# Research-Implementation/AudioVidSum-A-Multi-Modal-Approach-to-Video-Summarization

Measured on AMD Instinct MI355X. Metric: frames/sec end-to-end (extract+fuse+score), 224x224 + 16kHz, higher is better.
Workload: dtype f16x2; 1 GPU; configs[1]: SumMe-shape batch, 25 videos x ~1800 frames (45143 frames/GPU), visual-only resnet50 extractor (batch-stat BN, the reference's 4-frame BatchNorm micro-batches inside each video) + AVBiLSTM attention scorer + mean-threshold selection; frames_per_gpu=45143, videos_per_gpu=25, extractor=resnet50, frames_per_group=4, chunk_frames=16384, parallelism=videos sharded x1, no data-path collective, selected_frames_rank0=22823

## Files before the change

### audiovidsum-a-multi-modal-approach-to-video-summarization_amd/_abi.py

```python
import ctypes
import os
from ctypes import POINTER, c_char_p, c_double, c_float, c_int, c_int64, c_size_t, c_uint, c_void_p

import torch

_PKG_DIR = os.path.dirname(os.path.abspath(__file__))
STUDY = os.environ.get("AVS_STUDY_LIB") == "1"
_FLAVOUR = os.environ.get("AVS_STUDY_LIB")
LIB_PATH = os.path.join(_PKG_DIR, "lib", "libavsum_hip_study.so" if STUDY else
                        "libavsum_hip_fp16emu.so" if _FLAVOUR == "fp16emu" else "libavsum_hip.so")
HEADER_PATH = os.path.join(os.path.dirname(_PKG_DIR), "include", "avsum_hip.h")

AVS_F32, AVS_BF16, AVS_F32_ACC64, AVS_F32_SPLIT, AVS_F16X2 = 0, 1, 2, 3, 4
AVS_W_ROWS, AVS_W_KSTEP32 = 0, 1
TILE_AUTO, TILE_128, TILE_256, TILE_224, STAGING_GENERIC = 0, 1, 2, 3, 4
X_F16P8, Y_F16P8, RES_F16P8 = 1, 2, 4
LSTM_AUTO, LSTM_STREAM, LSTM_RESIDENT_20_8, LSTM_RESIDENT_16_8 = 0, 1, 2, 3
LSTM_SPLIT4 = 4
ACT_NONE, ACT_RELU = 0, 1
BIAS_NONE, BIAS_COL, BIAS_ROW = 0, 1, 2
E_UNSUPPORTED = -6


class AvsError(RuntimeError):
    pass


class ConvDesc(ctypes.Structure):
    _fields_ = [
        ("dtype", c_int),
        ("n", c_int), ("h", c_int), ("w", c_int),
        ("cin", c_int), ("kh", c_int), ("kw", c_int),
        ("sh", c_int), ("sw", c_int), ("ph", c_int), ("pw", c_int),
        ("ho", c_int), ("wo", c_int), ("cout", c_int),
        ("x_img_stride", c_int64), ("x_row_stride", c_int64), ("x_px_stride", c_int64),
        ("w_row_stride", c_int64), ("y_px_stride", c_int64),
        ("act", c_int), ("alpha", c_float), ("w_layout", c_int), ("variant", c_int), ("formats", c_int),
    ]


P = c_void_p
_SIGNATURES = {
    "avs_abi_version": (c_int, []),
    "avs_last_error": (c_char_p, []),
    "avs_device_info": (c_int, [c_int, POINTER(c_int), POINTER(c_int), POINTER(c_int64), c_char_p, c_int]),
    "avs_f16x2_pack_f32": (c_int, [P, P, c_int64, P]),
    "avs_f16x2_unpack_f32": (c_int, [P, P, c_int64, P]),
    "avs_f16p8_pack_f32": (c_int, [P, P, c_int64, P]),
# ... 77 lines not shown
    "avs_lstm_split_f32": (c_int, [P, P, c_int, c_int, c_uint, P, c_int, P, c_int64, c_int, P, P, P, c_size_t, c_uint, P]),
    "avs_lstm_bwd_split_f32": (c_int, [P, c_int64, c_int, P, P, P, c_int, c_int, c_uint, P, c_int, P, P, c_size_t, c_uint, P]),
    "avs_cdist_f64": (c_int, [P, c_int, P, c_int, c_int, P, P]),
    "avs_dtw_workspace_bytes": (c_int64, [c_int, c_int]),
    "avs_dtw_path_f64": (c_int, [P, c_int, c_int, P, c_int64, P, P, P, P]),
    "avs_gather_scale_f32": (c_int, [P, c_int64, c_int, P, P, c_int, P, P]),
}

_lib = None


def declared_symbols():
    import re
    text = open(HEADER_PATH).read()
    text = re.sub(r"/\*.*?\*/", "", text, flags=re.S)
    return sorted(set(re.findall(r"\b(avs_[a-z0-9_]+)\s*\(", text)))


def lib():
    global _lib
    if _lib is not None:
        return _lib
    if not os.path.exists(LIB_PATH):
        raise AvsError(
            f"{LIB_PATH} is missing: the HIP extension has not been built "
            "(run __graft_entry__.build() or `make -C <package>/csrc`). There is no CPU fallback."
        )
    handle = ctypes.CDLL(LIB_PATH)
    if STUDY:
        handle.avs_debug_flags.restype = None
        handle.avs_debug_flags.argtypes = [c_int]
        for name, args in (("avs_tune_short_reduction_bytes", [c_int]), ("avs_tune_tall_rule", [c_int, c_int]),
                           ("avs_tune_pipeline", [c_int]), ("avs_tune_bnlocal", [c_int]),
                           ("avs_tune_convbn_narrow", [c_int])):
            getattr(handle, name).restype = None
            getattr(handle, name).argtypes = args
    for name, (res, args) in _SIGNATURES.items():
        fn = getattr(handle, name)
        fn.restype = res
        fn.argtypes = args
    if handle.avs_abi_version() != 5:
        raise AvsError(f"ABI version mismatch: library reports {handle.avs_abi_version()}, binding expects 5")
    if STUDY and os.environ.get("AVS_TUNE_CONVBN_NARROW") is not None:
        handle.avs_tune_convbn_narrow(int(os.environ["AVS_TUNE_CONVBN_NARROW"]))
    if STUDY and os.environ.get("AVS_TUNE_PIPELINE") is not None:
        handle.avs_tune_pipeline(int(os.environ["AVS_TUNE_PIPELINE"]))
    _lib = handle
    return _lib


def check(status, what):
    if status != 0:
        msg = lib().avs_last_error()
        raise AvsError(f"{what} failed with status {status}: {msg.decode() if msg else ''}")


def device_info(dev=0):
    cu, clk, mem = c_int(), c_int(), c_int64()
    arch = ctypes.create_string_buffer(64)
    check(lib().avs_device_info(dev, ctypes.byref(cu), ctypes.byref(clk), ctypes.byref(mem), arch, 64),
          "avs_device_info")
    return {"cu_count": cu.value, "clock_khz": clk.value, "hbm_bytes": mem.value, "arch": arch.value.decode()}
```

### audiovidsum-a-multi-modal-approach-to-video-summarization_amd/csrc/igemm.hip

```cpp
#include "avs_internal.h"
#include "igemm_params.h"
#include <type_traits>

__device__ __attribute__((aligned(16))) unsigned int avs_zero16[4];

#ifdef AVS_STUDY
#define AVS_DEBUG_BIT(p, bit) ((p).debug & (bit))
#else
#define AVS_DEBUG_BIT(p, bit) 0
#endif

#define AVS_GLDS16(src, dst)                                                                        \
  __builtin_amdgcn_global_load_lds((const __attribute__((address_space(1))) void*)(src),            \
                                   (__attribute__((address_space(3))) void*)(dst), 16, 0, 0)

__device__ __forceinline__ void avs_split_bf16(const float4& p0, const float4& p1, bf16x8& hi, bf16x8& lo) {
  const float v[8] = {p0.x, p0.y, p0.z, p0.w, p1.x, p1.y, p1.z, p1.w};
  unsigned h[4], l[4];
#pragma unroll
  for (int j = 0; j < 4; ++j) {
    const unsigned short h0 = avs_f32_to_bf16(v[2 * j]), h1 = avs_f32_to_bf16(v[2 * j + 1]);
    const unsigned short l0 = avs_f32_to_bf16(v[2 * j] - avs_bf16_to_f32(h0));
    const unsigned short l1 = avs_f32_to_bf16(v[2 * j + 1] - avs_bf16_to_f32(h1));
    h[j] = (unsigned)h0 | ((unsigned)h1 << 16);
// ... 1414 lines not shown
            v = (float)(acc64[mt][nt][e] * (double)p.alpha) + bcol;
          else if constexpr (EPI == EPI_ANY)
            v = fmaf(acc[mt][nt][e], p.alpha, bcol);
          else if constexpr (EPI == EPI_BRELU)
            v = fmaxf(acc[mt][nt][e] + bcol, 0.f);
          else
            v = acc[mt][nt][e];
          if constexpr (EPI == EPI_ANY) {
            if (p.bias_mode == AVS_BIAS_ROW) v += bias[row];
            if (p.act == AVS_ACT_RELU) v = fmaxf(v, 0.f);
          }
          *reinterpret_cast<float*>(y + ((long long)row * p.ldc + col) * 4) = v;
        }
      }
    stats_fold();
  }
  }
}

#ifdef AVS_STUDY
static int g_debug_flags = 0;
extern "C" void avs_debug_flags(int flags) { g_debug_flags = flags; }
#endif
#ifdef AVS_STUDY
#define AVS_RULE static int
#else
#define AVS_RULE static constexpr int
#endif
AVS_RULE g_rowb_threshold_bytes = 2048;
AVS_RULE g_tall_min_tiles = 2048;
AVS_RULE g_tall_min_k_bytes = 1024;
AVS_RULE g_pipe3 = 1;
AVS_RULE g_bnlocal = 1;
static constexpr int AVS_RULE_AFFINE_128_MAX_K = 128;
#ifdef AVS_STUDY
extern "C" void avs_tune_short_reduction_bytes(int bytes) { g_rowb_threshold_bytes = bytes; }
extern "C" void avs_tune_tall_rule(int min_tiles, int min_k_bytes) {
  if (min_tiles > 0) g_tall_min_tiles = min_tiles;
  if (min_k_bytes >= 0) g_tall_min_k_bytes = min_k_bytes;
}
extern "C" void avs_tune_pipeline(int enabled) { g_pipe3 = enabled; }
extern "C" void avs_tune_bnlocal(int enabled) { g_bnlocal = enabled; }
#endif

static bool igemm_tap9_ok(const IgemmParams& p, int es) {
  return (p.variant & 3) != AVS_TILE_256 && p.KW == 3 && p.K == 9 * p.cin && p.sh == 1 && p.sw == 1 && p.ph == 1 && p.pw == 1 &&
         p.W <= 63 && p.HoWo == p.H * p.W && p.Wo == p.W && p.x_px_stride == p.cin &&
         p.x_row_stride == (long long)p.W * p.cin && p.x_img_stride == (long long)p.HoWo * p.cin && p.cin % (64 / es) == 0 &&
         (long long)(384 + 64) * p.cin * es < (1ll << 31);
}

static bool igemm_taps_ok(const IgemmParams& p) {
  if ((p.variant & 3) == AVS_TILE_256 || p.cin <= 0 || p.KW <= 0 || p.K % (p.cin * p.KW) != 0) return false;
  const int kh = p.K / (p.cin * p.KW);
  return kh * p.KW > 1 && kh * p.KW <= 32 && p.sh == 1 && p.sw == 1 && 2 * p.ph + 1 == kh && 2 * p.pw + 1 == p.KW &&
         p.HoWo == p.H * p.W && p.Wo == p.W && p.ph * p.W + p.pw <= 64 && p.x_px_stride >= p.cin &&
         p.x_row_stride == (long long)p.W * p.x_px_stride && p.x_img_stride == (long long)p.HoWo * p.x_px_stride &&
         p.cin % 16 == 0 && (long long)(384 + 64) * p.x_px_stride * 4 + (long long)p.cin * 4 < (1ll << 31);
}

#define AVS_LAUNCH_RET(K)                                     \
  do {                                                        \
    hipLaunchKernelGGL(K, grid, dim3(256), 0, stream, p);     \
    return true;                                              \
  } while (0)
template <int ES, int BN, bool ACC64, bool SP, int ROWB, bool PIPE, int WR, bool FK>
static bool igemm_dispatch_epi4(int epi, dim3 grid, hipStream_t stream, const IgemmParams& p) {
  if (p.in_scale) {
    if constexpr (ES == 4 && !ACC64 && SP && ROWB == 64 && PIPE && WR == 4 && FK) {
      if (p.split == 2 && epi == EPI_STATS && igemm_tap9_ok(p, ES))
        AVS_LAUNCH_RET((igemm_kernel<ES, BN, ACC64, SP, ROWB, EPI_STATS, PIPE, WR, FK, 2, true, false, true>));
    }
    return false;
  }
  if constexpr (ES == 2 && WR == 4) {
// ... 249 lines not shown
                    p.x_img_stride == (long long)p.HoWo * p.x_px_stride && p.x_px_stride % 16 == 0 &&
                    256 * p.x_px_stride * 3 + (long long)p.K * 3 < (1ll << 31),
                AVS_E_UNSUPPORTED,
                "%s: an AVS_F16P8 input is taken by avs_conv2d_nhwc_bnstats for 1x1 / stride-1 convolutions on dense rows, "
                "cin a multiple of 32 (>= 64), the input row stride a multiple of 16", who);
  }
  if (p.affine) {
    const int tile_mode = p.variant & 3;
    p.tall = (!narrow && (tile_mode == AVS_TILE_128 || (tile_mode == AVS_TILE_AUTO && p.K <= AVS_RULE_AFFINE_128_MAX_K))) ? 0 : 1;
    if (!p.tall && (long long)p.K * 4 > g_rowb_threshold_bytes) p.tall = 1;
  }
  const int tile_rows = p.tile_rows ? p.tile_rows : (p.tall ? 256 : 128);
  const long long tiles_m = ((long long)p.M + tile_rows - 1) / tile_rows;
  const long long total = tiles_m * p.tiles_n;
  AVS_REQUIRE(total < (1ll << 31), AVS_E_SHAPE, "%s: too many tiles", who);
  if (tiles_m_out) *tiles_m_out = tiles_m;
  if (plan_only) return AVS_OK;
  const bool spatial = !(p.ph == 0 && p.pw == 0 && (p.HoWo / p.Wo - 1) * p.sh + (p.K / (p.cin * p.KW)) - 1 < p.H &&
                         (p.Wo - 1) * p.sw + p.KW - 1 < p.W);
  p.lin_stride = -1;
  if (!spatial && p.KW == 1 && p.K == p.cin && p.sh == 1 && p.sw == 1) {
    if (p.HoWo == 1)
      p.lin_stride = p.x_img_stride;
    else if (p.x_row_stride == (long long)p.Wo * p.x_px_stride && p.x_img_stride == (long long)p.HoWo * p.x_px_stride)
      p.lin_stride = p.x_px_stride;
  }
  dim3 grid((unsigned)total, 1, (unsigned)batch);
  if (p.tile_rows && dtype == AVS_F16X2) {
    const bool fits = igemm_h2_local224_ok(p, dtype);
    AVS_REQUIRE(fits || p.cluster <= 1, AVS_E_UNSUPPORTED, "%s: the clustered form runs on the 224-row tile only", who);
    AVS_REQUIRE(fits || (p.variant & 3) != AVS_TILE_224, AVS_E_UNSUPPORTED,
                "%s: AVS_TILE_224 takes AVS_F16X2, groups of 193..224 rows, cout in multiples of 128, cin in multiples of 16", who);
    if (fits) {
      igemm_h2_local224_launch(p, spatial, grid, stream);
      AVS_CHECK_LAUNCH(who);
      return AVS_OK;
    }
  }
  bool launched;
  if (wide96) {
    launched = igemm_dispatch_brelu96(spatial, grid, stream, p);
  } else if (dtype == AVS_BF16) {
    launched = narrow ? igemm_dispatch<2, 64, false>(spatial, grid, stream, p) : igemm_dispatch<2, 128, false>(spatial, grid, stream, p);
  } else if (dtype == AVS_F32_ACC64) {
    launched = igemm_dispatch<4, 64, true>(spatial, grid, stream, p);
  } else {
    launched = narrow ? igemm_dispatch<4, 64, false>(spatial, grid, stream, p) : igemm_dispatch<4, 128, false>(spatial, grid, stream, p);
  }
  AVS_REQUIRE(launched, AVS_E_UNSUPPORTED,
              "%s: no kernel for this combination (dtype %d, %s tile, K = %d, N = %d, variant %d, %s%s%s): nothing was launched", who,
              dtype, p.tall ? "256-row" : "128-row", p.K, p.N, p.variant, p.affine ? "given-affine " : "", p.tile_rows ? "tile-local " : "",
              p.stat_part ? "statistics" : "");
  AVS_CHECK_LAUNCH(who);
  return AVS_OK;
}

static int conv_fill_params(const avs_conv_desc* d, const void* d_x, const void* d_w, const float* d_bias, void* d_y,
                            IgemmParams& p, const char* who) {
  AVS_REQUIRE(d != nullptr, AVS_E_ARG, "%s: null descriptor", who);
  AVS_REQUIRE(d->n >= 0 && d->h > 0 && d->w > 0 && d->cin > 0 && d->kh > 0 && d->kw > 0 && d->sh > 0 && d->sw > 0 &&
                  d->ph >= 0 && d->pw >= 0 && d->ho > 0 && d->wo > 0 && d->cout > 0,
              AVS_E_SHAPE, "%s: non-positive extent", who);
  AVS_REQUIRE((d->ho - 1) * d->sh - d->ph + d->kh - 1 < d->h + d->ph &&
                  (d->wo - 1) * d->sw - d->pw + d->kw - 1 < d->w + d->pw,
              AVS_E_SHAPE, "%s: output extent %dx%d exceeds what input %dx%d allows", who, d->ho, d->wo, d->h, d->w);
  const long long rows = (long long)d->n * d->ho * d->wo;
  AVS_REQUIRE(rows < (1ll << 31), AVS_E_SHAPE, "%s: %lld output pixels exceed int32", who, rows);
  p.x = (const char*)d_x;
  p.w = (const char*)d_w;
  p.y = (char*)d_y;
  p.bias = d_bias;
  p.M = (int)rows;
  p.N = d->cout;
  p.K = d->kh * d->kw * d->cin;
  p.HoWo = d->ho * d->wo;
  p.Wo = d->wo;
  p.H = d->h;
  p.W = d->w;
  p.cin = d->cin;
  p.KW = d->kw;
  p.sh = d->sh;
  p.sw = d->sw;
  p.ph = d->ph;
  p.pw = d->pw;
  p.x_img_stride = d->x_img_stride;
  p.x_row_stride = d->x_row_stride;
  p.x_px_stride = d->x_px_stride;
  p.ldb = d->w_row_stride;
  AVS_REQUIRE(d->w_layout == AVS_W_ROWS || d->w_layout == AVS_W_KSTEP32, AVS_E_ARG, "%s: bad w_layout %d", who,
              d->w_layout);
  p.w_kstep = d->w_layout == AVS_W_KSTEP32 ? 1 : 0;
  AVS_REQUIRE((d->variant & ~7) == 0, AVS_E_ARG, "%s: bad variant %d", who, d->variant);
  p.variant = d->variant;
  AVS_REQUIRE((d->formats & ~(AVS_X_F16P8 | AVS_Y_F16P8 | AVS_RES_F16P8)) == 0, AVS_E_ARG, "%s: bad formats %d", who, d->formats);
  AVS_REQUIRE(d->formats == 0 || d->dtype == AVS_F16X2, AVS_E_UNSUPPORTED, "%s: AVS_F16P8 operands belong to the AVS_F16X2 forms", who);
  p.x_p8 = (d->formats & AVS_X_F16P8) ? 1 : 0;
  p.y_p8 = (d->formats & AVS_Y_F16P8) ? 1 : 0;
  p.res_p8 = (d->formats & AVS_RES_F16P8) ? 1 : 0;
  AVS_REQUIRE(!p.w_kstep || (d->dtype != AVS_F32_ACC64 && p.K % (d->dtype == AVS_BF16 ? 32 : 16) == 0), AVS_E_UNSUPPORTED,
              "%s: the reduction-step-major weight layout needs a reduction that is a multiple of a 64-byte step (K = %d)",
              who, p.K);
  p.ldc = d->y_px_stride;
  p.alpha = d->alpha;
  p.act = d->act;
  p.bias_mode = d_bias ? AVS_BIAS_COL : AVS_BIAS_NONE;
  AVS_REQUIRE(p.ldb >= p.K, AVS_E_SHAPE, "%s: w_row_stride %lld < kh*kw*cin=%d", who, p.ldb, p.K);
  return AVS_OK;
}

extern "C" int avs_conv2d_nhwc(const avs_conv_desc* d, const void* d_x, const void* d_w, const float* d_bias,
                               void* d_y, avs_stream_t stream) {
  IgemmParams p{};
  int st = conv_fill_params(d, d_x, d_w, d_bias, d_y, p, "avs_conv2d_nhwc");
  if (st != AVS_OK) return st;
  return igemm_launch(d->dtype, p, 1, (hipStream_t)stream, "avs_conv2d_nhwc");
}

extern "C" int avs_conv2d_nhwc_split(const avs_conv_desc* d, const void* d_x, const void* d_w, const float* d_bias,
                                     void* d_y, int n_split, void* d_y2, int64_t y2_px_stride, int relu_cols,
                                     avs_stream_t stream) {
  const char* who = "avs_conv2d_nhwc_split";
  IgemmParams p{};
  int st = conv_fill_params(d, d_x, d_w, d_bias, d_y, p, who);
  if (st != AVS_OK) return st;
  AVS_REQUIRE(d->dtype == AVS_F16X2, AVS_E_UNSUPPORTED, "%s: built for AVS_F16X2", who);
// ... 342 lines not shown
```

### audiovidsum-a-multi-modal-approach-to-video-summarization_amd/csrc/igemm_params.h

```cpp
#pragma once
#include "avs_internal.h"

typedef __bf16 bf16x8 __attribute__((ext_vector_type(8)));
typedef float f32x16 __attribute__((ext_vector_type(16)));

struct IgemmParams {
  const char* x;
  const char* w;
  char* y;
  const float* bias;
  int M, N, K;
  int HoWo, Wo, H, W, cin, KW;
  int sh, sw, ph, pw;
  long long x_img_stride, x_row_stride, x_px_stride;
  long long ldb, ldc;
  long long sA, sB, sC, sBias;
  float alpha;
  int act, bias_mode;
  int tiles_n;
  float* stat_part;
  int stat_slots;
  int rows_per_group;
  long long lin_stride;
  const float* gamma;
  const float* beta;
  float eps;
  const char* residual;
  long long ldr;
  int split;
  int tall;
  int w_kstep;
  int tile_rows;
  int affine;
  const float* res_scale;
  const float* res_shift;
  int variant;
  int x_p8, y_p8, res_p8;
  char* y2;
  long long ldc2;
  int nsplit;
  int relu_cols;
  int cluster;
  unsigned epoch;
  unsigned long long* xchg;
  unsigned* xerr;
  const float* in_scale;
  const float* in_shift;
  int in_relu;
#ifdef AVS_STUDY
  int debug;
#endif
};

enum { EPI_PLAIN = 0, EPI_STATS = 1, EPI_ANY = 2, EPI_BRELU = 3, EPI_BNLOCAL = 5, EPI_AFFINE = 6 };
constexpr int BNLOCAL_MAX_GROUPS = 6;
constexpr int STATS_MIN_GROUP_ROWS = 64;

typedef unsigned u32x4 __attribute__((ext_vector_type(4)));
typedef unsigned u32x2 __attribute__((ext_vector_type(2)));
__device__ __forceinline__ void avs_pin(uint4& v) {
  u32x4 r = __builtin_bit_cast(u32x4, v);
  asm volatile("" : "+v"(r));
  v = __builtin_bit_cast(uint4, r);
}

__device__ __forceinline__ void avs_pin2(uint2& v) {
  u32x2 r = __builtin_bit_cast(u32x2, v);
  asm volatile("" : "+v"(r));
  v = __builtin_bit_cast(uint2, r);
}
__device__ __forceinline__ uint2 avs_lds_read_b64(unsigned byte_addr) {
  uint2 v;
  asm volatile("ds_read_b64 %0, %1" : "=v"(v) : "v"(byte_addr));
  return v;
}
__device__ __forceinline__ uint4 avs_lds_read_b128(unsigned byte_addr) {
  uint4 v;
  asm volatile("ds_read_b128 %0, %1" : "=v"(v) : "v"(byte_addr));
// ... 7 lines not shown
```

### audiovidsum-a-multi-modal-approach-to-video-summarization_amd/csrc/local224.hip

```cpp
#include "avs_internal.h"
#include "igemm_params.h"
#include <type_traits>
#include <utility>

namespace {
constexpr int L_ROWS = 224;
constexpr int L_MT = L_ROWS / 32;
constexpr int L_BN = 128;
constexpr int L_CPRR = 4;
constexpr int L_STEP = 16;
constexpr int L_BUF = (L_ROWS + L_BN) * L_CPRR;
constexpr int L_P = 32 + 8;
constexpr unsigned L_OOB = 0x80000000u;

template <int OFF>
__device__ __forceinline__ uint4 lds_read_b128_at(unsigned byte_addr) {
  uint4 v;
  asm volatile("ds_read_b128 %0, %1 offset:%2" : "=v"(v) : "v"(byte_addr), "n"(OFF));
  return v;
}
template <int... I>
__device__ __forceinline__ void read_blocks(uint4 (&f)[L_MT], unsigned addr, std::integer_sequence<int, I...>) {
  ((f[I] = lds_read_b128_at<I * 32 * 64>(addr)), ...);
}
}

template <bool SPATIAL>
__global__ __launch_bounds__(256, 2) void igemm_h2_local224_kernel(IgemmParams p) {
  __shared__ uint4 lds[3 * L_BUF];

  const unsigned nwg = gridDim.x, orig = blockIdx.x;
  const unsigned q = nwg >> 3, rr = nwg & 7, xcd = orig & 7;
  const unsigned wg = (xcd < rr ? xcd * (q + 1) : rr * (q + 1) + (xcd - rr) * q) + (orig >> 3);
  int tn = wg % p.tiles_n;
  int tm = wg / p.tiles_n;
  if (p.cluster > 1) {
    const unsigned c = (unsigned)p.cluster, tnn = (unsigned)p.tiles_n;
    const unsigned tiles_m = nwg / tnn;
    const unsigned full = (8u % c == 0u) ? (tiles_m / 8u) * 8u : 0u;
    if (orig < full * tnn) {
      const unsigned su = orig / (8u * tnn), l = orig - su * (8u * tnn);
      tn = (int)(l >> 3);
      tm = (int)(su * 8u + (l & 7u));
    } else {
      const unsigned o2 = orig - full * tnn, unit = c * tnn;
      const unsigned u = o2 / unit, l = o2 - u * unit;
      tn = (int)(l / c);
      tm = (int)(full + u * c + l % c);
    }
  }
  const int m0 = tm * p.tile_rows;
  const int n0 = tn * L_BN;
  const int used = m0 + p.tile_rows <= p.M ? p.tile_rows : p.M - m0;

  const char* __restrict__ x = p.x;
  const char* __restrict__ w = p.w;
  char* __restrict__ y = p.y;

  const int t = threadIdx.x;
  const int wave = __builtin_amdgcn_readfirstlane(t >> 6), lane = t & 63;
  const bool extra = wave < 2;
  const int c = t & (L_CPRR - 1);
  const int rb = t >> 2;
  const int cq = c ^ ((rb >> 2) & (L_CPRR - 1));

  unsigned amask[4], aoff[4], boff[2];
  int f_tap = 0, f_ci0 = 0, f_kw = 0;
  int f_koff = 0;
  int f_kb = 0;
  __amdgpu_buffer_rsrc_t a_rsrc, b_rsrc;
  {
    const int taps = p.K / p.cin;
    long long a_origin;
    int n_first = 0;
    if (p.lin_stride >= 0) {
      a_origin = (long long)m0 * p.lin_stride;
    } else {
      n_first = m0 / p.HoWo;
      a_origin = (long long)n_first * p.x_img_stride - (long long)p.ph * p.x_row_stride - (long long)p.pw * p.x_px_stride;
    }
    a_rsrc = __builtin_amdgcn_make_buffer_rsrc(const_cast<char*>(x) + a_origin * 4, 0, (int)L_OOB, 0x00020000);
    b_rsrc = __builtin_amdgcn_make_buffer_rsrc(
        const_cast<char*>(w) + (p.w_kstep ? (long long)n0 * 64 : (long long)n0 * p.ldb * 4), 0, (int)L_OOB, 0x00020000);
#pragma unroll
    for (int i = 0; i < 4; ++i) {
      unsigned mk = 0, off = L_OOB;
      const int r = rb + 64 * i;
      if (r < used) {
        const int m = m0 + r;
        if (p.lin_stride >= 0) {
          mk = ~0u;
          off = (unsigned)((long long)r * p.lin_stride * 4) + cq * 16;
        } else {
          const int n = m / p.HoWo;
          const int rem = m - n * p.HoWo;
          const int ho = rem / p.Wo;
          const int wo = rem - ho * p.Wo;
          const int hi0 = ho * p.sh - p.ph, wi0 = wo * p.sw - p.pw;
          if constexpr (SPATIAL) {
            for (int tp = 0; tp < taps; ++tp) {
              const int th = tp / p.KW, tw = tp - th * p.KW;
              if ((unsigned)(hi0 + th) < (unsigned)p.H && (unsigned)(wi0 + tw) < (unsigned)p.W) mk |= 1u << tp;
            }
          } else {
            mk = ~0u;
          }
          off = (unsigned)(((long long)(n - n_first) * p.x_img_stride + (long long)(hi0 + p.ph) * p.x_row_stride +
                            (long long)(wi0 + p.pw) * p.x_px_stride) * 4) + cq * 16;
        }
      }
      amask[i] = mk;
      aoff[i] = off;
    }
#pragma unroll
    for (int i = 0; i < 2; ++i)
      boff[i] = p.w_kstep ? (unsigned)((rb + 64 * i) * 64) + (unsigned)(cq >> 2) * (unsigned)p.N * 64u + (cq & 3) * 16
                          : (unsigned)((long long)(rb + 64 * i) * p.ldb * 4) + cq * 16;
  }

  auto stage = [&](int buf) {
    uint4* abuf = lds + buf * L_BUF + wave * 64;
    uint4* bbuf = abuf + L_ROWS * L_CPRR;
#pragma unroll
    for (int i = 0; i < 3; ++i) {
      unsigned off = aoff[i];
      if constexpr (SPATIAL) off = ((amask[i] >> f_tap) & 1u) ? off : L_OOB;
      __builtin_amdgcn_raw_ptr_buffer_load_lds(a_rsrc, (__attribute__((address_space(3))) void*)(abuf + 256 * i), 16,
                                               (int)off, f_koff, 0, 0);
    }
    if (extra) {
      unsigned off = aoff[3];
      if constexpr (SPATIAL) off = ((amask[3] >> f_tap) & 1u) ? off : L_OOB;
      __builtin_amdgcn_raw_ptr_buffer_load_lds(a_rsrc, (__attribute__((address_space(3))) void*)(abuf + 256 * 3), 16,
                                               (int)off, f_koff, 0, 0);
    }
#pragma unroll
    for (int i = 0; i < 2; ++i)
      __builtin_amdgcn_raw_ptr_buffer_load_lds(b_rsrc, (__attribute__((address_space(3))) void*)(bbuf + 256 * i), 16,
                                               (int)boff[i], f_kb, 0, 0);
    f_kb += p.w_kstep ? p.N * 64 : L_STEP * 4;
    f_ci0 += L_STEP;
    f_koff += L_STEP * 4;
    if (f_ci0 == p.cin) {
      f_ci0 = 0;
      ++f_tap;
      f_koff += (int)((p.x_px_stride - p.cin) * 4);
      if (++f_kw == p.KW) {
        f_kw = 0;
        f_koff += (int)((p.x_row_stride - (long long)p.KW * p.x_px_stride) * 4);
      }
    }
  };

  const int lr = lane & 31, lh = lane >> 5;

  f32x16 acc[L_MT];
#pragma unroll
  for (int i = 0; i < L_MT; ++i)
#pragma unroll
    for (int e = 0; e < 16; ++e) acc[i][e] = 0.f;

  const unsigned lds_base = (unsigned)(unsigned long long)((__attribute__((address_space(3))) char*)lds);
  unsigned fa_off[2], fb_off[2];
#pragma unroll
  for (int hl = 0; hl < 2; ++hl) {
    const int chunk = 2 * lh + hl;
    fa_off[hl] = (unsigned)(lr * L_CPRR + (chunk ^ ((lr >> 2) & (L_CPRR - 1)))) * 16u;
    const int brow = wave * 32 + lr;
    fb_off[hl] = (unsigned)((L_ROWS + brow) * L_CPRR + (chunk ^ ((brow >> 2) & (L_CPRR - 1)))) * 16u;
  }

  const int col = n0 + wave * 32 + lr;
  const float inv_n = 1.f / (float)p.tile_rows;
  const int lim = used - 4 * lh;
  const int rl0 = lane >> 2, grp = lane & 3;
  const int col8 = n0 + wave * 32 + grp * 8;
  constexpr int DEPTH = 6;
  uint4 rhi[DEPTH][2], rlo[DEPTH][2];
  auto res_fetch = [&](auto blk) {
    constexpr int mt = decltype(blk)::value;
    const long long row0 = (long long)m0 + mt * 32 + rl0;
    const char* base = p.residual + (row0 * p.ldr + col8) * 4;
#pragma unroll
    for (int it = 0; it < 2; ++it) {
      const bool ok = mt * 32 + rl0 + 16 * it < used;
      const uint4* rp = reinterpret_cast<const uint4*>(ok ? base + (long long)it * 16 * p.ldr * 4 : p.residual);
      rhi[mt % DEPTH][it] = rp[0];
      rlo[mt % DEPTH][it] = rp[1];
    }
  };
  if (p.residual) {
    res_fetch(std::integral_constant<int, 0>{});
    res_fetch(std::integral_constant<int, 1>{});
    res_fetch(std::integral_constant<int, 2>{});
  }

  const int steps = p.K / L_STEP;
  stage(0);
  if (steps > 1) stage(1);
  int cur = 0;
  for (int s = 0; s < steps; ++s) {
    if (s + 1 < steps) {
      if (extra)
        asm volatile("s_waitcnt vmcnt(6)" ::: "memory");
      else
        asm volatile("s_waitcnt vmcnt(5)" ::: "memory");
    } else {
      asm volatile("s_waitcnt vmcnt(0)" ::: "memory");
    }
    __builtin_amdgcn_s_barrier();
    const unsigned bbase = lds_base + (unsigned)cur * (L_BUF * 16u);
    uint4 fah[L_MT], fal[L_MT], fbh, fbl;
    fbh = avs_lds_read_b128(bbase + fb_off[0]);
    read_blocks(fah, bbase + fa_off[0], std::make_integer_sequence<int, L_MT>{});
    fbl = avs_lds_read_b128(bbase + fb_off[1]);
    read_blocks(fal, bbase + fa_off[1], std::make_integer_sequence<int, L_MT>{});
    if (s + 2 < steps) stage(cur == 0 ? 2 : cur - 1);
    asm volatile("s_waitcnt lgkmcnt(%0)" ::"n"(1 + L_MT) : "memory");
    avs_pin(fbh);
#pragma unroll
    for (int mt = 0; mt < L_MT; ++mt) avs_pin(fah[mt]);
    __builtin_amdgcn_sched_barrier(0);
#pragma unroll
    for (int mt = 0; mt < L_MT; ++mt)
      acc[mt] = __builtin_amdgcn_mfma_f32_32x32x16_f16(__builtin_bit_cast(avs_f16x8, fah[mt]),
                                                       __builtin_bit_cast(avs_f16x8, fbh), acc[mt], 0, 0, 0);
    asm volatile("s_waitcnt lgkmcnt(0)" ::: "memory");
    avs_pin(fbl);
#pragma unroll
    for (int mt = 0; mt < L_MT; ++mt) avs_pin(fal[mt]);
    __builtin_amdgcn_sched_barrier(0);
#pragma unroll
    for (int mt = 0; mt < L_MT; ++mt) {
      acc[mt] = __builtin_amdgcn_mfma_f32_32x32x16_f16(__builtin_bit_cast(avs_f16x8, fal[mt]),
                                                       __builtin_bit_cast(avs_f16x8, fbh), acc[mt], 0, 0, 0);
      acc[mt] = __builtin_amdgcn_mfma_f32_32x32x16_f16(__builtin_bit_cast(avs_f16x8, fah[mt]),
                                                       __builtin_bit_cast(avs_f16x8, fbl), acc[mt], 0, 0, 0);
    }
    __builtin_amdgcn_sched_barrier(0);
    cur = cur == 2 ? 0 : cur + 1;
  }

  if (p.residual) {
    res_fetch(std::integral_constant<int, 3>{});
    res_fetch(std::integral_constant<int, 4>{});
    res_fetch(std::integral_constant<int, 5>{});
  }
  float s1 = 0.f;
#pragma unroll
  for (int mt = 0; mt < L_MT; ++mt)
#pragma unroll
    for (int e = 0; e < 16; ++e) s1 += acc[mt][e];
  s1 += __shfl_xor(s1, 32, 64);
  const float mean = s1 * inv_n;
  float s2 = 0.f;
#pragma unroll
  for (int mt = 0; mt < L_MT; ++mt)
#pragma unroll
    for (int e = 0; e < 16; ++e) {
      const int roff = mt * 32 + (e & 3) + 8 * (e >> 2);
      const float d = acc[mt][e] - mean;
      s2 = roff < lim ? fmaf(d, d, s2) : s2;
    }
  s2 += __shfl_xor(s2, 32, 64);
  float g_mean = mean, g_var = s2 * inv_n;
  if (p.cluster > 1) {
    const int cj = tm % p.cluster, t0 = tm - cj;
    unsigned long long* slot = p.xchg + (((long long)tm * p.tiles_n + tn) * 4 + wave) * 64 + lane;
    const float mine = lh ? s2 : mean;
    __hip_atomic_store(slot, ((unsigned long long)p.epoch << 32) | (unsigned long long)__float_as_uint(mine), __ATOMIC_RELAXED,
                       __HIP_MEMORY_SCOPE_AGENT);
    const float nt = (float)p.tile_rows;
    float n = 0.f, mu = 0.f, m2 = 0.f;
    const unsigned long long* const gbase = p.xchg + (((long long)t0 * p.tiles_n + tn) * 4 + wave) * 64 + lane;
    const long long gstride = (long long)p.tiles_n * 4 * 64;
    for (int j0 = 0; j0 < p.cluster; j0 += 4) {
      unsigned long long g[4];
#pragma unroll
      for (int u = 0; u < 4; ++u) {
        const int j = j0 + u < p.cluster ? j0 + u : cj;
        g[u] = __hip_atomic_load(gbase + j * gstride, __ATOMIC_RELAXED, __HIP_MEMORY_SCOPE_AGENT);
      }
#pragma unroll
      for (int u = 0; u < 4; ++u) {
        const int j = j0 + u;
        if (j >= p.cluster) break;
        float mj = mean, qj = s2;
        if (j != cj) {
          bool ok = (unsigned)(g[u] >> 32) == p.epoch;
          for (int spin = 0; spin < (1 << 20) && __builtin_amdgcn_read_exec() != __builtin_amdgcn_ballot_w64(ok); ++spin) {
            __builtin_amdgcn_s_sleep(8);
            g[u] = __hip_atomic_load(gbase + j * gstride, __ATOMIC_RELAXED, __HIP_MEMORY_SCOPE_AGENT);
            ok = (unsigned)(g[u] >> 32) == p.epoch;
          }
          if (__builtin_amdgcn_read_exec() != __builtin_amdgcn_ballot_w64(ok) && lane == 0) atomicAdd(p.xerr, 1u);
          const float v = __uint_as_float((unsigned)g[u]);
          const float o = __shfl_xor(v, 32, 64);
          mj = lh ? o : v;
          qj = lh ? v : o;
        }
        const float tot = n + nt, delta = mj - mu;
        mu += delta * (nt / tot);
        m2 += qj + delta * delta * (n * nt / tot);
        n = tot;
      }
    }
    g_mean = mu;
    g_var = m2 / n;
  }
  const float sc = p.gamma[col] / sqrtf(g_var + p.eps);
  const float sf = p.beta[col] - g_mean * sc;
#pragma unroll
  for (int mt = 0; mt < L_MT; ++mt)
#pragma unroll
    for (int e = 0; e < 16; ++e) acc[mt][e] = fmaf(acc[mt][e], sc, sf);
  const bool relu = p.act == AVS_ACT_RELU;

  __syncthreads();
  float* const wreg = reinterpret_cast<float*>(lds) + wave * (32 * L_P);
  auto emit = [&](auto blk) {
    constexpr int mt = decltype(blk)::value;
#pragma unroll
    for (int e = 0; e < 16; ++e) wreg[((e & 3) + 8 * (e >> 2) + 4 * lh) * L_P + lr] = acc[mt][e];
    asm volatile("s_waitcnt lgkmcnt(0)" ::: "memory");
    __builtin_amdgcn_wave_barrier();
    const long long row0 = (long long)m0 + mt * 32 + rl0;
    char* const ybase = y + (row0 * p.ldc + col8) * 4;
#pragma unroll
    for (int it = 0; it < 2; ++it) {
      const float* src = wreg + (rl0 + 16 * it) * L_P + grp * 8;
      const float4 f0 = *reinterpret_cast<const float4*>(src);
      const float4 f1 = *reinterpret_cast<const float4*>(src + 4);
      if (!(mt * 32 + rl0 + 16 * it < used)) continue;
      float v[8] = {f0.x, f0.y, f0.z, f0.w, f1.x, f1.y, f1.z, f1.w};
      if (p.residual) {
        float rv[8];
        avs_pin(rhi[mt % DEPTH][it]);
        avs_pin(rlo[mt % DEPTH][it]);
        avs_f16x2_join8(rhi[mt % DEPTH][it], rlo[mt % DEPTH][it], rv);
#pragma unroll
        for (int j = 0; j < 8; ++j) v[j] += rv[j];
      }
      if (relu) {
#pragma unroll
        for (int j = 0; j < 8; ++j) v[j] = fmaxf(v[j], 0.f);
      }
      uint4 hi, lo;
      avs_f16x2_split8(v, hi, lo);
      uint4* dst = reinterpret_cast<uint4*>(ybase + (long long)it * 16 * p.ldc * 4);
      dst[0] = hi;
      dst[1] = lo;
    }
    asm volatile("s_waitcnt lgkmcnt(0)" ::: "memory");
    __builtin_amdgcn_wave_barrier();
    if constexpr (mt + DEPTH < L_MT) {
      if (p.residual) res_fetch(std::integral_constant<int, mt + DEPTH>{});
    }
  };
  emit(std::integral_constant<int, 0>{});
  emit(std::integral_constant<int, 1>{});
  emit(std::integral_constant<int, 2>{});
  emit(std::integral_constant<int, 3>{});
  emit(std::integral_constant<int, 4>{});
  emit(std::integral_constant<int, 5>{});
  emit(std::integral_constant<int, 6>{});
}

bool igemm_h2_local224_ok(const IgemmParams& p, int dtype) {
  const int tile_mode = p.variant & 3;
  if (dtype != AVS_F16X2 || !(tile_mode == AVS_TILE_AUTO || tile_mode == AVS_TILE_224)) return false;
  if (p.variant & AVS_STAGING_GENERIC) return false;
  const int cl = p.cluster > 1 ? p.cluster : 1;
  if (p.tile_rows * cl != p.rows_per_group || p.tile_rows <= 192 || p.tile_rows > L_ROWS) return false;
  if (p.N % L_BN != 0 || p.M % p.rows_per_group != 0) return false;
  if (p.cin % L_STEP != 0 || p.K % L_STEP != 0 || p.K % p.cin != 0 || p.K / p.cin > 32) return false;
  const long long rows = 256;
  long long extent;
  if (p.lin_stride >= 0)
    extent = rows * p.lin_stride + p.K;
  else
    extent = (rows / p.HoWo + 2) * p.x_img_stride + (long long)(p.K / (p.cin * p.KW) + p.ph) * p.x_row_stride +
             (long long)(p.KW + p.pw) * p.x_px_stride + p.cin;
  return extent * 4 < (1ll << 31) && (long long)L_BN * p.ldb * 4 + (long long)p.K * 4 < (1ll << 31) &&
         p.x_img_stride >= 0 && p.x_row_stride >= 0 && p.x_px_stride >= 0;
}

void igemm_h2_local224_launch(const IgemmParams& p, bool spatial, dim3 grid, hipStream_t stream) {
  if (spatial)
    hipLaunchKernelGGL(igemm_h2_local224_kernel<true>, grid, dim3(256), 0, stream, p);
  else
    hipLaunchKernelGGL(igemm_h2_local224_kernel<false>, grid, dim3(256), 0, stream, p);
}
```

### include/avsum_hip.h

```cpp
#ifndef AVSUM_HIP_H
#define AVSUM_HIP_H

#include <stdint.h>

#ifdef __cplusplus
extern "C" {
#endif

#define AVS_ABI_VERSION 5

enum {
  AVS_OK = 0,
  AVS_E_ARG = -1,
  AVS_E_SHAPE = -2,
  AVS_E_ALIGN = -3,
  AVS_E_HIP = -4,
  AVS_E_WORKSPACE = -5,
  AVS_E_UNSUPPORTED = -6
};

enum { AVS_F32 = 0, AVS_BF16 = 1, AVS_F32_ACC64 = 2, AVS_F32_SPLIT = 3, AVS_F16X2 = 4 };
enum { AVS_ACT_NONE = 0, AVS_ACT_RELU = 1 };
enum { AVS_BIAS_NONE = 0, AVS_BIAS_COL = 1, AVS_BIAS_ROW = 2 };

typedef void* avs_stream_t;

int avs_abi_version(void);
const char* avs_last_error(void);
int avs_device_info(int dev, int* cu_count, int* clock_khz, int64_t* hbm_bytes,
                    char* arch, int arch_len);

int avs_f16x2_pack_f32(const float* d_src, void* d_dst, int64_t n, avs_stream_t stream);
int avs_f16x2_unpack_f32(const void* d_src, float* d_dst, int64_t n, avs_stream_t stream);

int avs_f16p8_pack_f32(const float* d_src, void* d_dst, int64_t n, avs_stream_t stream);
int avs_f16p8_unpack_f32(const void* d_src, float* d_dst, int64_t n, avs_stream_t stream);


typedef struct {
  int dtype;
  int n, h, w;
  int cin, kh, kw;
  int sh, sw, ph, pw;
  int ho, wo, cout;
  int64_t x_img_stride;
  int64_t x_row_stride;
  int64_t x_px_stride;
  int64_t w_row_stride;
  int64_t y_px_stride;
  int act;
  float alpha;
  int w_layout;
  int variant;
  int formats;
} avs_conv_desc;
enum { AVS_W_ROWS = 0, AVS_W_KSTEP32 = 1 };
enum { AVS_X_F16P8 = 1, AVS_Y_F16P8 = 2, AVS_RES_F16P8 = 4 };
enum { AVS_TILE_AUTO = 0, AVS_TILE_128 = 1, AVS_TILE_256 = 2, AVS_TILE_224 = 3, AVS_STAGING_GENERIC = 4 };

int avs_conv2d_nhwc(const avs_conv_desc* desc, const void* d_x, const void* d_w,
                    const float* d_bias, void* d_y, avs_stream_t stream);
int avs_conv2d_nhwc_split(const avs_conv_desc* desc, const void* d_x, const void* d_w, const float* d_bias, void* d_y,
                          int n_split, void* d_y2, int64_t y2_px_stride, int relu_cols, avs_stream_t stream);

int64_t avs_conv2d_bnstats_workspace_bytes(const avs_conv_desc* desc, int64_t rows_per_group);
int avs_conv2d_nhwc_bnstats(const avs_conv_desc* desc, const void* d_x, const void* d_w, void* d_y,
                            int64_t rows_per_group, const float* d_gamma, const float* d_beta, float eps,
                            float* d_scale, float* d_shift, void* d_ws, int64_t ws_bytes, avs_stream_t stream);
int avs_conv2d_nhwc_bnstats_xin(const avs_conv_desc* desc, const void* d_x, const void* d_w, void* d_y,
                                int64_t rows_per_group, const float* d_gamma, const float* d_beta, float eps,
                                float* d_scale, float* d_shift, void* d_ws, int64_t ws_bytes, const float* d_in_scale,
                                const float* d_in_shift, int in_relu, avs_stream_t stream);

int avs_conv2d_bnlocal_tile_rows(const avs_conv_desc* desc, int64_t rows_per_group);
int avs_conv2d_nhwc_bnlocal(const avs_conv_desc* desc, const void* d_x, const void* d_w, void* d_y,
                            int64_t rows_per_group, const float* d_gamma, const float* d_beta, float eps,
                            const void* d_residual, int64_t ldr, avs_stream_t stream);

int64_t avs_conv2d_bncluster_workspace_bytes(const avs_conv_desc* desc, int64_t rows_per_group, int cluster);
int avs_conv2d_nhwc_bncluster(const avs_conv_desc* desc, const void* d_x, const void* d_w, void* d_y,
                              int64_t rows_per_group, int cluster, const float* d_gamma, const float* d_beta, float eps,
                              const void* d_residual, int64_t ldr, void* d_xchg, int64_t xchg_bytes, uint32_t epoch,
                              avs_stream_t stream);
int avs_bn_gram_affine_f16x2(const void* d_x, int64_t lin_stride, int k, const float* d_in_scale,
                             const float* d_in_shift, const void* d_w, int64_t ldb, int n, int64_t rows_per_group,
                             int groups, const float* d_gamma, const float* d_beta, float eps, float* d_scale,
                             float* d_shift, void* d_a_out, int64_t lda, avs_stream_t stream);
int avs_conv2d_nhwc_affine(const avs_conv_desc* desc, const void* d_x, const void* d_w, void* d_y,
                           int64_t rows_per_group, const float* d_scale, const float* d_shift,
                           const void* d_residual, int64_t ldr, const float* d_res_scale, const float* d_res_shift,
                           avs_stream_t stream);
// ... 199 lines not shown
```

Baseline: 27360 frames/s.

## Walk multiple N tiles per workgroup in local224 conv-BN kernel

The local224 fused conv+batch-stat BN kernel can now have each workgroup process several consecutive output-column tiles, keeping the A-side row tile resident. It prefetches the next tile's weights during the tail of the current K loop, so staging overlaps the epilogue and per-workgroup prologue costs are amortised. The walk length is chosen from the CU count so enough workgroups remain (at least 12 rounds of 2 per CU). The residual path becomes a template parameter and the residual prefetch depth is reduced, lowering register pressure. The trade-off is fewer, longer workgroups, with a risk of tail imbalance and more complex wait-count logic.

Measured after the change: 27060 frames/s. 1.1% lower.

```diff
diff --git a/audiovidsum-a-multi-modal-approach-to-video-summarization_amd/_abi.py b/audiovidsum-a-multi-modal-approach-to-video-summarization_amd/_abi.py
--- a/audiovidsum-a-multi-modal-approach-to-video-summarization_amd/_abi.py
+++ b/audiovidsum-a-multi-modal-approach-to-video-summarization_amd/_abi.py
@@ -14,6 +14,7 @@
 AVS_F32, AVS_BF16, AVS_F32_ACC64, AVS_F32_SPLIT, AVS_F16X2 = 0, 1, 2, 3, 4
 AVS_W_ROWS, AVS_W_KSTEP32 = 0, 1
 TILE_AUTO, TILE_128, TILE_256, TILE_224, STAGING_GENERIC = 0, 1, 2, 3, 4
+WALK_OFF, WALK_FULL = 8, 16
 X_F16P8, Y_F16P8, RES_F16P8 = 1, 2, 4
 LSTM_AUTO, LSTM_STREAM, LSTM_RESIDENT_20_8, LSTM_RESIDENT_16_8 = 0, 1, 2, 3
 LSTM_SPLIT4 = 4
@@ -157,7 +158,7 @@
         handle.avs_debug_flags.argtypes = [c_int]
         for name, args in (("avs_tune_short_reduction_bytes", [c_int]), ("avs_tune_tall_rule", [c_int, c_int]),
                            ("avs_tune_pipeline", [c_int]), ("avs_tune_bnlocal", [c_int]),
-                           ("avs_tune_convbn_narrow", [c_int])):
+                           ("avs_tune_convbn_narrow", [c_int]), ("avs_tune_walk_rounds", [c_int])):
             getattr(handle, name).restype = None
             getattr(handle, name).argtypes = args
     for name, (res, args) in _SIGNATURES.items():
diff --git a/audiovidsum-a-multi-modal-approach-to-video-summarization_amd/csrc/igemm.hip b/audiovidsum-a-multi-modal-approach-to-video-summarization_amd/csrc/igemm.hip
--- a/audiovidsum-a-multi-modal-approach-to-video-summarization_amd/csrc/igemm.hip
+++ b/audiovidsum-a-multi-modal-approach-to-video-summarization_amd/csrc/igemm.hip
@@ -1470,6 +1470,7 @@
 AVS_RULE g_tall_min_k_bytes = 1024;
 AVS_RULE g_pipe3 = 1;
 AVS_RULE g_bnlocal = 1;
+AVS_RULE g_walk_min_rounds = 12;
 static constexpr int AVS_RULE_AFFINE_128_MAX_K = 128;
 #ifdef AVS_STUDY
 extern "C" void avs_tune_short_reduction_bytes(int bytes) { g_rowb_threshold_bytes = bytes; }
@@ -1479,6 +1480,7 @@
 }
 extern "C" void avs_tune_pipeline(int enabled) { g_pipe3 = enabled; }
 extern "C" void avs_tune_bnlocal(int enabled) { g_bnlocal = enabled; }
+extern "C" void avs_tune_walk_rounds(int rounds) { if (rounds > 0) g_walk_min_rounds = rounds; }
 #endif
 
 static bool igemm_tap9_ok(const IgemmParams& p, int es) {
@@ -1794,6 +1796,24 @@
     AVS_REQUIRE(fits || (p.variant & 3) != AVS_TILE_224, AVS_E_UNSUPPORTED,
                 "%s: AVS_TILE_224 takes AVS_F16X2, groups of 193..224 rows, cout in multiples of 128, cin in multiples of 16", who);
     if (fits) {
+      int walk = 1;
+      if (p.variant & AVS_WALK_FULL) {
+        walk = p.tiles_n;
+      } else if (!(p.variant & AVS_WALK_OFF) && p.tiles_n > 1 && p.cluster <= 1) {
+        int dev = 0, cus = 0;
+        AVS_REQUIRE(hipGetDevice(&dev) == hipSuccess &&
+                        hipDeviceGetAttribute(&cus, hipDeviceAttributeMultiprocessorCount, dev) == hipSuccess && cus > 0,
+                    AVS_E_HIP, "%s: cannot read the device's CU count", who);
+        const long long slots = 2ll * cus;
+        for (int d = p.tiles_n; d > 1; --d)
+          if (p.tiles_n % d == 0 && tiles_m * (p.tiles_n / d) >= (long long)g_walk_min_rounds * slots) {
+            walk = d;
+            break;
+          }
+      }
+      p.walk = walk;
+      p.walk_runs = p.tiles_n / walk;
+      grid.x = (unsigned)(tiles_m * p.walk_runs);
       igemm_h2_local224_launch(p, spatial, grid, stream);
       AVS_CHECK_LAUNCH(who);
       return AVS_OK;
@@ -1852,7 +1872,7 @@
   AVS_REQUIRE(d->w_layout == AVS_W_ROWS || d->w_layout == AVS_W_KSTEP32, AVS_E_ARG, "%s: bad w_layout %d", who,
               d->w_layout);
   p.w_kstep = d->w_layout == AVS_W_KSTEP32 ? 1 : 0;
-  AVS_REQUIRE((d->variant & ~7) == 0, AVS_E_ARG, "%s: bad variant %d", who, d->variant);
+  AVS_REQUIRE((d->variant & ~31) == 0 && (d->variant & (AVS_WALK_OFF | AVS_WALK_FULL)) != (AVS_WALK_OFF | AVS_WALK_FULL), AVS_E_ARG, "%s: bad variant %d", who, d->variant);
   p.variant = d->variant;
   AVS_REQUIRE((d->formats & ~(AVS_X_F16P8 | AVS_Y_F16P8 | AVS_RES_F16P8)) == 0, AVS_E_ARG, "%s: bad formats %d", who, d->formats);
   AVS_REQUIRE(d->formats == 0 || d->dtype == AVS_F16X2, AVS_E_UNSUPPORTED, "%s: AVS_F16P8 operands belong to the AVS_F16X2 forms", who);
diff --git a/audiovidsum-a-multi-modal-approach-to-video-summarization_amd/csrc/igemm_params.h b/audiovidsum-a-multi-modal-approach-to-video-summarization_amd/csrc/igemm_params.h
--- a/audiovidsum-a-multi-modal-approach-to-video-summarization_amd/csrc/igemm_params.h
+++ b/audiovidsum-a-multi-modal-approach-to-video-summarization_amd/csrc/igemm_params.h
@@ -44,6 +44,7 @@
   unsigned epoch;
   unsigned long long* xchg;
   unsigned* xerr;
+  int walk, walk_runs;
   const float* in_scale;
   const float* in_shift;
   int in_relu;
diff --git a/audiovidsum-a-multi-modal-approach-to-video-summarization_amd/csrc/local224.hip b/audiovidsum-a-multi-modal-approach-to-video-summarization_amd/csrc/local224.hip
--- a/audiovidsum-a-multi-modal-approach-to-video-summarization_amd/csrc/local224.hip
+++ b/audiovidsum-a-multi-modal-approach-to-video-summarization_amd/csrc/local224.hip
@@ -25,32 +25,34 @@
 }
 }
 
-template <bool SPATIAL>
+template <bool SPATIAL, bool RES>
 __global__ __launch_bounds__(256, 2) void igemm_h2_local224_kernel(IgemmParams p) {
   __shared__ uint4 lds[3 * L_BUF];
 
   const unsigned nwg = gridDim.x, orig = blockIdx.x;
   const unsigned q = nwg >> 3, rr = nwg & 7, xcd = orig & 7;
   const unsigned wg = (xcd < rr ? xcd * (q + 1) : rr * (q + 1) + (xcd - rr) * q) + (orig >> 3);
-  int tn = wg % p.tiles_n;
-  int tm = wg / p.tiles_n;
+  const unsigned runs = (unsigned)p.walk_runs;
+  int run = wg % runs;
+  int tm = wg / runs;
   if (p.cluster > 1) {
-    const unsigned c = (unsigned)p.cluster, tnn = (unsigned)p.tiles_n;
-    const unsigned tiles_m = nwg / tnn;
+    const unsigned c = (unsigned)p.cluster;
+    const unsigned tiles_m = nwg / runs;
     const unsigned full = (8u % c == 0u) ? (tiles_m / 8u) * 8u : 0u;
-    if (orig < full * tnn) {
-      const unsigned su = orig / (8u * tnn), l = orig - su * (8u * tnn);
-      tn = (int)(l >> 3);
+    if (orig < full * runs) {
+      const unsigned su = orig / (8u * runs), l = orig - su * (8u * runs);
+      run = (int)(l >> 3);
       tm = (int)(su * 8u + (l & 7u));
     } else {
-      const unsigned o2 = orig - full * tnn, unit = c * tnn;
+      const unsigned o2 = orig - full * runs, unit = c * runs;
       const unsigned u = o2 / unit, l = o2 - u * unit;
-      tn = (int)(l / c);
+      run = (int)(l / c);
       tm = (int)(full + u * c + l % c);
     }
   }
+  const int walk = p.walk;
+  int tn = run * walk;
   const int m0 = tm * p.tile_rows;
-  const int n0 = tn * L_BN;
   const int used = m0 + p.tile_rows <= p.M ? p.tile_rows : p.M - m0;
 
   const char* __restrict__ x = p.x;
@@ -69,6 +71,11 @@
   int f_koff = 0;
   int f_kb = 0;
   __amdgpu_buffer_rsrc_t a_rsrc, b_rsrc;
+  auto b_window = [&](int ct) {
+    const long long nb = (long long)ct * L_BN;
+    return __builtin_amdgcn_make_buffer_rsrc(const_cast<char*>(w) + (p.w_kstep ? nb * 64 : nb * p.ldb * 4), 0, (int)L_OOB,
+                                             0x00020000);
+  };
   {
     const int taps = p.K / p.cin;
     long long a_origin;
@@ -80,8 +87,7 @@
       a_origin = (long long)n_first * p.x_img_stride - (long long)p.ph * p.x_row_stride - (long long)p.pw * p.x_px_stride;
     }
     a_rsrc = __builtin_amdgcn_make_buffer_rsrc(const_cast<char*>(x) + a_origin * 4, 0, (int)L_OOB, 0x00020000);
-    b_rsrc = __builtin_amdgcn_make_buffer_rsrc(
-        const_cast<char*>(w) + (p.w_kstep ? (long long)n0 * 64 : (long long)n0 * p.ldb * 4), 0, (int)L_OOB, 0x00020000);
+    b_rsrc = b_window(tn);
 #pragma unroll
     for (int i = 0; i < 4; ++i) {
       unsigned mk = 0, off = L_OOB;
@@ -112,11 +118,15 @@
       amask[i] = mk;
       aoff[i] = off;
     }
+  }
+  auto set_boff = [&](int tid) {
+    const int r0 = tid >> 2, q0 = (tid & (L_CPRR - 1)) ^ ((r0 >> 2) & (L_CPRR - 1));
 #pragma unroll
     for (int i = 0; i < 2; ++i)
-      boff[i] = p.w_kstep ? (unsigned)((rb + 64 * i) * 64) + (unsigned)(cq >> 2) * (unsigned)p.N * 64u + (cq & 3) * 16
-                          : (unsigned)((long long)(rb + 64 * i) * p.ldb * 4) + cq * 16;
-  }
+      boff[i] = p.w_kstep ? (unsigned)((r0 + 64 * i) * 64) + (unsigned)(q0 >> 2) * (unsigned)p.N * 64u + (q0 & 3) * 16
+                          : (unsigned)((long long)(r0 + 64 * i) * p.ldb * 4) + q0 * 16;
+  };
+  set_boff(t);
 
   auto stage = [&](int buf) {
     uint4* abuf = lds + buf * L_BUF + wave * 64;
@@ -152,15 +162,23 @@
     }
   };
 
-  const int lr = lane & 31, lh = lane >> 5;
-
-  f32x16 acc[L_MT];
-#pragma unroll
-  for (int i = 0; i < L_MT; ++i)
-#pragma unroll
-    for (int e = 0; e < 16; ++e) acc[i][e] = 0.f;
-
   const unsigned lds_base = (unsigned)(unsigned long long)((__attribute__((address_space(3))) char*)lds);
+  const float inv_n = 1.f / (float)p.tile_rows;
+  const bool relu = p.act == AVS_ACT_RELU;
+  const int steps = p.K / L_STEP;
+
+  stage(0);
+  stage(1);
+  int cur = 0;
+#pragma nounroll
+  for (int j = 0; j < walk; ++j, ++tn) {
+  const bool more = j + 1 < walk;
+  const int n0 = tn * L_BN;
+  int lane_j = lane;
+  asm volatile("" : "+v"(lane_j));
+  const int lr = lane_j & 31, lh = lane_j >> 5;
+  const int lim = used - 4 * lh;
+  const int rl0 = lane_j >> 2, grp = lane_j & 3;
   unsigned fa_off[2], fb_off[2];
 #pragma unroll
   for (int hl = 0; hl < 2; ++hl) {
@@ -169,13 +187,18 @@
     const int brow = wave * 32 + lr;
     fb_off[hl] = (unsigned)((L_ROWS + brow) * L_CPRR + (chunk ^ ((brow >> 2) & (L_CPRR - 1)))) * 16u;
   }
+  if (j > 0) set_boff(wave * 64 + lane_j);
+
+  f32x16 acc[L_MT];
+#pragma unroll
+  for (int i = 0; i < L_MT; ++i)
+#pragma unroll
+    for (int e = 0; e < 16; ++e) acc[i][e] = 0.f;
 
   const int col = n0 + wave * 32 + lr;
-  const float inv_n = 1.f / (float)p.tile_rows;
-  const int lim = used - 4 * lh;
-  const int rl0 = lane >> 2, grp = lane & 3;
   const int col8 = n0 + wave * 32 + grp * 8;
-  constexpr int DEPTH = 6;
+  constexpr int DEPTH = SPATIAL ? 4 : 5;
+  constexpr int PRE = SPATIAL ? 2 : 3;
   uint4 rhi[DEPTH][2], rlo[DEPTH][2];
   auto res_fetch = [&](auto blk) {
     constexpr int mt = decltype(blk)::value;
@@ -189,24 +212,22 @@
       rlo[mt % DEPTH][it] = rp[1];
     }
   };
-  if (p.residual) {
+  if constexpr (RES) {
     res_fetch(std::integral_constant<int, 0>{});
     res_fetch(std::integral_constant<int, 1>{});
-    res_fetch(std::integral_constant<int, 2>{});
-  }
-
-  const int steps = p.K / L_STEP;
-  stage(0);
-  if (steps > 1) stage(1);
-  int cur = 0;
+    if constexpr (PRE > 2) res_fetch(std::integral_constant<int, 2>{});
+  }
+
   for (int s = 0; s < steps; ++s) {
-    if (s + 1 < steps) {
-      if (extra)
-        asm volatile("s_waitcnt vmcnt(6)" ::: "memory");
-      else
-        asm volatile("s_waitcnt vmcnt(5)" ::: "memory");
-    } else {
-      asm volatile("s_waitcnt vmcnt(0)" ::: "memory");
+    if (j == 0 || s >= 2) {
+      if (s + 1 < steps || more) {
+        if (extra)
+          asm volatile("s_waitcnt vmcnt(6)" ::: "memory");
+        else
+          asm volatile("s_waitcnt vmcnt(5)" ::: "memory");
+      } else {
+        asm volatile("s_waitcnt vmcnt(0)" ::: "memory");
+      }
     }
     __builtin_amdgcn_s_barrier();
     const unsigned bbase = lds_base + (unsigned)cur * (L_BUF * 16u);
@@ -215,7 +236,15 @@
     read_blocks(fah, bbase + fa_off[0], std::make_integer_sequence<int, L_MT>{});
     fbl = avs_lds_read_b128(bbase + fb_off[1]);
     read_blocks(fal, bbase + fa_off[1], std::make_integer_sequence<int, L_MT>{});
-    if (s + 2 < steps) stage(cur == 0 ? 2 : cur - 1);
+    if (s + 2 < steps) {
+      stage(cur == 0 ? 2 : cur - 1);
+    } else if (more) {
+      if (s + 2 == steps) {
+        f_tap = f_ci0 = f_kw = f_koff = f_kb = 0;
+        b_rsrc = b_window(tn + 1);
+      }
+      stage(cur == 0 ? 2 : cur - 1);
+    }
     asm volatile("s_waitcnt lgkmcnt(%0)" ::"n"(1 + L_MT) : "memory");
     avs_pin(fbh);
 #pragma unroll
@@ -240,11 +269,12 @@
     __builtin_amdgcn_sched_barrier(0);
     cur = cur == 2 ? 0 : cur + 1;
   }
-
-  if (p.residual) {
+  const int last = cur == 0 ? 2 : cur - 1;
+
+  if constexpr (RES) {
+    if constexpr (PRE < 3) res_fetch(std::integral_constant<int, 2>{});
     res_fetch(std::integral_constant<int, 3>{});
-    res_fetch(std::integral_constant<int, 4>{});
-    res_fetch(std::integral_constant<int, 5>{});
+    if constexpr (DEPTH > 4) res_fetch(std::integral_constant<int, 4>{});
   }
   float s1 = 0.f;
 #pragma unroll
@@ -266,13 +296,13 @@
   float g_mean = mean, g_var = s2 * inv_n;
   if (p.cluster > 1) {
     const int cj = tm % p.cluster, t0 = tm - cj;
-    unsigned long long* slot = p.xchg + (((long long)tm * p.tiles_n + tn) * 4 + wave) * 64 + lane;
+    unsigned long long* slot = p.xchg + (((long long)tm * p.tiles_n + tn) * 4 + wave) * 64 + lane_j;
     const float mine = lh ? s2 : mean;
     __hip_atomic_store(slot, ((unsigned long long)p.epoch << 32) | (unsigned long long)__float_as_uint(mine), __ATOMIC_RELAXED,
                        __HIP_MEMORY_SCOPE_AGENT);
     const float nt = (float)p.tile_rows;
     float n = 0.f, mu = 0.f, m2 = 0.f;
-    const unsigned long long* const gbase = p.xchg + (((long long)t0 * p.tiles_n + tn) * 4 + wave) * 64 + lane;
+    const unsigned long long* const gbase = p.xchg + (((long long)t0 * p.tiles_n + tn) * 4 + wave) * 64 + lane_j;
     const long long gstride = (long long)p.tiles_n * 4 * 64;
     for (int j0 = 0; j0 < p.cluster; j0 += 4) {
       unsigned long long g[4];
@@ -314,10 +344,12 @@
   for (int mt = 0; mt < L_MT; ++mt)
 #pragma unroll
     for (int e = 0; e < 16; ++e) acc[mt][e] = fmaf(acc[mt][e], sc, sf);
-  const bool relu = p.act == AVS_ACT_RELU;
-
-  __syncthreads();
-  float* const wreg = reinterpret_cast<float*>(lds) + wave * (32 * L_P);
+
+  asm volatile("" ::: "memory");
+  __builtin_amdgcn_s_waitcnt(0x0070);
+  __builtin_amdgcn_s_barrier();
+  asm volatile("" ::: "memory");
+  float* const wreg = reinterpret_cast<float*>(lds + last * L_BUF) + wave * (32 * L_P);
   auto emit = [&](auto blk) {
     constexpr int mt = decltype(blk)::value;
 #pragma unroll
@@ -333,7 +365,7 @@
       const float4 f1 = *reinterpret_cast<const float4*>(src + 4);
       if (!(mt * 32 + rl0 + 16 * it < used)) continue;
       float v[8] = {f0.x, f0.y, f0.z, f0.w, f1.x, f1.y, f1.z, f1.w};
-      if (p.residual) {
+      if constexpr (RES) {
         float rv[8];
         avs_pin(rhi[mt % DEPTH][it]);
         avs_pin(rlo[mt % DEPTH][it]);
@@ -354,7 +386,7 @@
     asm volatile("s_waitcnt lgkmcnt(0)" ::: "memory");
     __builtin_amdgcn_wave_barrier();
     if constexpr (mt + DEPTH < L_MT) {
-      if (p.residual) res_fetch(std::integral_constant<int, mt + DEPTH>{});
+      if constexpr (RES) res_fetch(std::integral_constant<int, mt + DEPTH>{});
     }
   };
   emit(std::integral_constant<int, 0>{});
@@ -364,6 +396,7 @@
   emit(std::integral_constant<int, 4>{});
   emit(std::integral_constant<int, 5>{});
   emit(std::integral_constant<int, 6>{});
+  }
 }
 
 bool igemm_h2_local224_ok(const IgemmParams& p, int dtype) {
@@ -374,6 +407,7 @@
   if (p.tile_rows * cl != p.rows_per_group || p.tile_rows <= 192 || p.tile_rows > L_ROWS) return false;
   if (p.N % L_BN != 0 || p.M % p.rows_per_group != 0) return false;
   if (p.cin % L_STEP != 0 || p.K % L_STEP != 0 || p.K % p.cin != 0 || p.K / p.cin > 32) return false;
+  if (p.K < 2 * L_STEP) return false;
   const long long rows = 256;
   long long extent;
   if (p.lin_stride >= 0)
@@ -386,8 +420,12 @@
 }
 
 void igemm_h2_local224_launch(const IgemmParams& p, bool spatial, dim3 grid, hipStream_t stream) {
-  if (spatial)
-    hipLaunchKernelGGL(igemm_h2_local224_kernel<true>, grid, dim3(256), 0, stream, p);
+  if (spatial && p.residual)
+    hipLaunchKernelGGL((igemm_h2_local224_kernel<true, true>), grid, dim3(256), 0, stream, p);
+  else if (spatial)
+    hipLaunchKernelGGL((igemm_h2_local224_kernel<true, false>), grid, dim3(256), 0, stream, p);
+  else if (p.residual)
+    hipLaunchKernelGGL((igemm_h2_local224_kernel<false, true>), grid, dim3(256), 0, stream, p);
   else
-    hipLaunchKernelGGL(igemm_h2_local224_kernel<false>, grid, dim3(256), 0, stream, p);
-}
+    hipLaunchKernelGGL((igemm_h2_local224_kernel<false, false>), grid, dim3(256), 0, stream, p);
+}
diff --git a/include/avsum_hip.h b/include/avsum_hip.h
--- a/include/avsum_hip.h
+++ b/include/avsum_hip.h
@@ -56,7 +56,8 @@
 } avs_conv_desc;
 enum { AVS_W_ROWS = 0, AVS_W_KSTEP32 = 1 };
 enum { AVS_X_F16P8 = 1, AVS_Y_F16P8 = 2, AVS_RES_F16P8 = 4 };
-enum { AVS_TILE_AUTO = 0, AVS_TILE_128 = 1, AVS_TILE_256 = 2, AVS_TILE_224 = 3, AVS_STAGING_GENERIC = 4 };
+enum { AVS_TILE_AUTO = 0, AVS_TILE_128 = 1, AVS_TILE_256 = 2, AVS_TILE_224 = 3, AVS_STAGING_GENERIC = 4,
+       AVS_WALK_OFF = 8, AVS_WALK_FULL = 16 };
 
 int avs_conv2d_nhwc(const avs_conv_desc* desc, const void* d_x, const void* d_w,
                     const float* d_bias, void* d_y, avs_stream_t stream);
```
